# MCG-NKU/E2FGVI

Hardware: AMD Instinct MI355X
Metric: inpainted frames/sec at 432x240 T=10 (higher is better)
Workload: dtype f32; 1 GPU; BASELINE.json configs[1]: e2fgvi 432x240 T=10 l_t=10, 1 clip(s) per GPU per forward (1 in the job), random-init weights, torch.rand frames + box mask (SURVEY.md 8d); clips_per_gpu=1, precision=fp32, kernel_selection=e2fgvi_amd/tile_table.py (checked in, deterministic: ops.py), hip_graph=True, forwards_in_flight=2

## Files before the change

e2fgvi_amd/build.py:

```python
import os
import subprocess
import sys
from concurrent.futures import ThreadPoolExecutor

HERE = os.path.dirname(os.path.abspath(__file__))
CSRC = os.path.join(HERE, "csrc")
LIB = os.path.join(CSRC, "libe2fgvi_hip.so")
FLAGS = ["--offload-arch=gfx950", "-O3", "-std=c++17", "-fPIC", "-ffp-contract=fast"]
NOPK = ["-Xclang", "-target-feature", "-Xclang", "-packed-fp32-ops"]
UNITS = [("error.hip", "error.o", []), ("conv.hip", "conv.o", []), ("conv.hip", "conv_nopk.o", NOPK + ["-DE2_NOPK_VARIANT"]),
         ("conv_bf16x.hip", "conv_bf16x.o", NOPK), ("conv_wino.hip", "conv_wino.o", NOPK), ("conv_wino.hip", "conv_wino_x3.o", NOPK + ["-DE2_WINO_X3=1"]), ("conv_wino4.hip", "conv_wino4.o", NOPK), ("conv_tail.hip", "conv_tail.o", NOPK),
         ("mdcn.hip", "mdcn.o", NOPK), ("attention.hip", "attention.o", []),
         ("attention_bf16.hip", "attention_bf16.o", NOPK), ("attention_x3.hip", "attention_x3.o", NOPK), ("misc.hip", "misc.o", NOPK),
         ("video.hip", "video.o", NOPK), ("metrics.hip", "metrics.o", NOPK)]
NOPK_OBJECTS = ("conv_nopk.o", "conv_bf16x.o", "conv_wino.o", "conv_wino4.o", "conv_wino_x3.o", "conv_tail.o", "mdcn.o", "attention_bf16.o", "attention_x3.o", "misc.o", "video.o", "metrics.o")
OBJDUMP = "/opt/rocm/lib/llvm/bin/llvm-objdump"


def _hipcc():
    for c in (os.environ.get("HIPCC"), "/opt/rocm/bin/hipcc"):
        if c and os.path.exists(c):
            return c
    return "hipcc"


def _stale(out, deps):
    return (not os.path.exists(out)) or any(os.path.getmtime(d) > os.path.getmtime(out) for d in deps)


def build(force=False, verbose=False, nopk_all=False, lib=None, tag=None, defines=()):
    hipcc = _hipcc()
    if tag:
        nopk_all = False
    objdir = os.path.join(CSRC, ("build_" + tag) if tag else ("build_nopk" if nopk_all else "build"))
    os.makedirs(objdir, exist_ok=True)
    out = lib or (os.path.join(CSRC, "libe2fgvi_hip_%s.so" % tag) if tag else
                  os.path.join(CSRC, "libe2fgvi_hip_nopk.so") if nopk_all else LIB)
    headers = [os.path.join(CSRC, "common.h"), os.path.join(HERE, "..", "include", "e2fgvi_hip.h"), os.path.abspath(__file__)]
    jobs = []
    for src, obj, extra in UNITS:
        sp, op = os.path.join(CSRC, src), os.path.join(objdir, obj)
        if nopk_all and not any(f == "-packed-fp32-ops" for f in extra):
            extra = extra + NOPK
        if force or _stale(op, [sp] + headers):
            jobs.append([hipcc] + FLAGS + extra + list(defines) + ["-c", sp, "-o", op])

    def run(cmd):
        if verbose:
            print(" ".join(cmd), flush=True)
        subprocess.check_call(cmd)

    with ThreadPoolExecutor(max_workers=min(4, max(1, len(jobs)))) as ex:
        list(ex.map(run, jobs))
    objs = [os.path.join(objdir, obj) for _, obj, _ in UNITS]
    if force or jobs or _stale(out, objs):
        run([hipcc, "--offload-arch=gfx950", "-shared", "-fPIC", "-o", out] + objs)
    if jobs:
        verify_isa(objdir)
        if not nopk_all:
            verify_wino_waits(objdir)
            verify_exit_reuse(objdir)
            verify_no_scratch(objdir)
    return out


def build_variant(tag, *defines):
    return build(tag=tag, defines=defines)


def device_isa(obj):
    import shutil
    import tempfile
    d = tempfile.mkdtemp(prefix="e2isa")
    try:
        local = os.path.join(d, os.path.basename(obj))
        shutil.copy(obj, local)
        subprocess.run([OBJDUMP, "--offloading", os.path.basename(obj)], cwd=d, check=True, stdout=subprocess.DEVNULL,
                       stderr=subprocess.DEVNULL)
        dev = [f for f in os.listdir(d) if "gfx950" in f]
        if not dev:
            return ""
        return subprocess.run([OBJDUMP, "-d", os.path.join(d, dev[0])], check=True, capture_output=True, text=True).stdout
    finally:
        shutil.rmtree(d, ignore_errors=True)


def verify_isa(objdir=None):
    import re
    objdir = objdir or os.path.join(CSRC, "build")
    if not os.path.exists(OBJDUMP):
        return
    for obj in NOPK_OBJECTS:
        isa = device_isa(os.path.join(objdir, obj))
# ... 84 lines not shown
                                       % (obj, name[:60], ins[a][0], ins[b][0]))
            g = counts[0] - counts[1] if len(counts) > 1 else counts[0]
            if counts[-1] != 0 or g <= 0 or any(c != counts[0] - j * g for j, c in enumerate(counts)):
                raise RuntimeError("%s: %s: group waits %s are not (P-1) G, ..., G, 0" % (obj, name[:60], counts))
            tail = [k for k in list(range(inner[-1] + 2, hi + 1)) + list(range(lo, inner[0])) if vmem.match(ins[k][1])]
            planes = tail[-(counts[0] + g):]
            if len(planes) != counts[0] + g or any(ins[k][1] != "buffer_load_dwordx4" or " lds" in ins[k][2] for k in planes):
                raise RuntimeError("%s: %s: the %d vector-memory instructions in front of the group waits are not the plane "
                                   "loads" % (obj, name[:60], counts[0] + g))
            continue
        for j, m in enumerate(inner):
            n = int(re.search(r"vmcnt\((\d+)\)", ins[m][2]).group(1))
            if j:
                rng = range(inner[j - 1] + 2, m)
            else:
                rng = list(range(inner[-1] + 2, hi + 1)) + list(range(lo, m))
            cnt = sum(1 for k in rng if vmem.match(ins[k][1]))
            if cnt != n:
                raise RuntimeError("%s: %s: explicit s_waitcnt vmcnt(%d) at 0x%x follows %d vector-memory instructions "
                                   "since the previous explicit wait" % (obj, name[:60], n, ins[m][0], cnt))
    return loops


def verify_wino_waits(objdir=None, objects=("conv_wino.o", "conv_wino_x3.o", "conv_wino4.o")):
    objdir = objdir or os.path.join(CSRC, "build")
    if not os.path.exists(OBJDUMP):
        return 0
    loops = 0
    for obj in objects:
        for name, ins in _kernels(device_isa(os.path.join(objdir, obj))).items():
            loops += check_kernel_waits(obj, name, ins)
    if not loops:
        raise RuntimeError("verify_wino_waits: no K loop with marked waits found (disassembly format changed?)")
    return loops


def _vregs(text):
    import re
    r = set()
    for m in re.finditer(r"\bv\[(\d+):(\d+)\]", text):
        r.update(range(int(m.group(1)), int(m.group(2)) + 1))
    for m in re.finditer(r"\bv(\d+)\b", text):
        r.add(int(m.group(1)))
    return r


def _successors(ins, at):
    succ = []
    for i, (a, m, o) in enumerate(ins):
        if m in ("s_endpgm", "s_endpgm_saved"):
            succ.append(())
        elif m == "s_branch" or m.startswith("s_cbranch"):
            off = int(o.split()[0])
            off -= 65536 if off > 32767 else 0
            tgt = at.get(a + 4 + 4 * off)
            if tgt is None:
                raise RuntimeError("branch at 0x%x leaves the kernel" % a)
            succ.append((tgt,) if m == "s_branch" else (tgt, i + 1))
        elif m.startswith("s_setpc") or m.startswith("s_swappc"):
            raise RuntimeError("indirect jump at 0x%x: control flow cannot be followed" % a)
        else:
            succ.append((i + 1,) if i + 1 < len(ins) else ())
    return succ


def check_exit_reuse(obj, name, ins, min_mfma=8):
# ... 125 lines not shown
```

e2fgvi_amd/csrc/conv_bf16x.hip:

```cpp
#include "common.h"

namespace {

typedef __bf16 bf16x8 __attribute__((ext_vector_type(8)));
typedef unsigned int u32x4 __attribute__((ext_vector_type(4)));
typedef __attribute__((address_space(3))) void lds_void;

struct ConvXParams {
    const void* src[E2FGVI_MAX_SRC];
    int ld[E2FGVI_MAX_SRC];
    int coff[E2FGVI_MAX_SRC];
    int cpg[E2FGVI_MAX_SRC];
    unsigned src_bytes[E2FGVI_MAX_SRC];
    int nsrc;
    int N, H, W, Ho, Wo, KH, KW, stride, pad;
    int padx;
    int osy, osx, opy, opx, oH, oW;
    int res_bcast;
    int Cout, Cout_g, Npad;
    int M;
    int tilesM, tilesN;
    int nsteps;
    unsigned wgroup_bytes;
    long long wgroup_elems;
    const void* w;
    const float* bias;
    const void* res;
    int res_ld, res_coff, res_bf16;
    void* dst;
    int dst_ld, dst_coff, dst_bf16, dst_nchw;
    __bf16* dst2;
    int dst2_ld, dst2_coff;
    int split_from;
// ... 643 lines not shown
                for (int c = 0; c < 8; ++c) if (full || n + c < p.Cout_g) o[(long long)c * HoWo] = v[c];
            } else if (p.dst_bf16) {
                E16* o = reinterpret_cast<E16*>(p.dst) + dof;
                if (vec_d) *reinterpret_cast<e16x8*>(o) = hv;
                else {
#pragma unroll
                    for (int c = 0; c < 8; ++c) if (full || n + c < p.Cout_g) o[c] = hv[c];
                }
            } else {
                float* o = reinterpret_cast<float*>(p.dst) + dof;
                if (vec_d) {
                    f32x4 w0 = {v[0], v[1], v[2], v[3]}, w1 = {v[4], v[5], v[6], v[7]};
                    *reinterpret_cast<f32x4*>(o) = w0;
                    *reinterpret_cast<f32x4*>(o + 4) = w1;
                } else {
#pragma unroll
                    for (int c = 0; c < 8; ++c) if (full || n + c < p.Cout_g) o[c] = v[c];
                }
            }
            if (p.dst2 && !p.split_plane) {
                E16* o = reinterpret_cast<E16*>(p.dst2) + (long long)m * p.dst2_ld + p.dst2_coff + co;
                if (vec_2) *reinterpret_cast<e16x8*>(o) = hv;
                else {
#pragma unroll
                    for (int c = 0; c < 8; ++c) if (full || n + c < p.Cout_g) o[c] = hv[c];
                }
            }
        }
    }
    }
#endif
}

struct PackX {
    int Cout, groups, KH, KW, nsrc;
    int cpg[E2FGVI_MAX_SRC];
    int Cout_g, Npad, Cin_g, steps_per_tap;
    int kc, ch;
    int tp_cq;
    long long total, wgroup_elems;
};

bool geometry_x(int Cout, int groups, int KH, int KW, int nsrc, const int32_t* cpg, PackX* q, bool f32 = false) {
    q->kc = f32 ? 32 : 64;
    q->ch = f32 ? 4 : 8;
    q->tp_cq = 0;
    if (Cout <= 0 || groups <= 0 || Cout % groups || KH <= 0 || KW <= 0 || nsrc < 1 || nsrc > E2FGVI_MAX_SRC) return false;
    q->Cout = Cout; q->groups = groups; q->KH = KH; q->KW = KW; q->nsrc = nsrc;
    q->Cout_g = Cout / groups;
    q->Npad = round_up(q->Cout_g, 32);
    q->Cin_g = 0;
    q->steps_per_tap = 0;
    for (int s = 0; s < E2FGVI_MAX_SRC; ++s) q->cpg[s] = 0;
    for (int s = 0; s < nsrc; ++s) {
        if (cpg[s] <= 0 || cpg[s] % q->ch) return false;
        q->cpg[s] = cpg[s];
        q->Cin_g += cpg[s];
        q->steps_per_tap += cdiv(cpg[s], q->kc);
    }
    q->wgroup_elems = (long long)KH * KW * q->steps_per_tap * q->kc * q->Npad;
    q->total = q->wgroup_elems * groups;
    return true;
}

__device__ __forceinline__ float pack_value(const float* __restrict__ w, const PackX& p, int g, int step, int koct, int n, int e) {
    if (p.tp_cq) {
// ... 58 lines not shown
    p.tilesM = cdiv(p.M, BM);
    p.tilesN = cdiv(p.Cout_g, BN);
    if constexpr (PP) {
        if (mode != 2 || p.tp_cq) {
            e2fgvi_set_error("conv2d_x: the ping-pong tiles (107, 108) are for the split-operand mode without tap-packed weights");
            return E2FGVI_EUNSUP;
        }
        hipLaunchKernelGGL((conv_bf16x_kernel<BM, BN, WGM, WGN, false, 2, true>), dim3(p.tilesM * p.tilesN, groups, 1), dim3(64 * WGM * WGN), 0, st, p);
        E2_LAUNCH_CHECK("conv2d_x");
        return 0;
    } else {
    if (S3 && !(p.KH == 3 && p.KW == 3 && p.stride == 1 && p.pad == 1)) {
        e2fgvi_set_error("conv2d_x: the row-shift tiles (11..17) are for 3x3 stride-1 pad-1 layers");
        return E2FGVI_EINVAL;
    }
    if (mode == 1 || mode == 2) {
        if constexpr (!S3) {
            if (mode == 2)
                hipLaunchKernelGGL((conv_bf16x_kernel<BM, BN, WGM, WGN, false, 2>), dim3(p.tilesM * p.tilesN, groups, 1), dim3(64 * WGM * WGN), 0, st, p);
            else
                hipLaunchKernelGGL((conv_bf16x_kernel<BM, BN, WGM, WGN, false, 1>), dim3(p.tilesM * p.tilesN, groups, 1), dim3(64 * WGM * WGN), 0, st, p);
        } else {
            e2fgvi_set_error("conv2d_x: the row-shift tiles (11..18) take bf16 operands only");
            return E2FGVI_EUNSUP;
        }
    } else if (mode == 3) {
        hipLaunchKernelGGL((conv_bf16x_kernel<BM, BN, WGM, WGN, S3, 3>), dim3(p.tilesM * p.tilesN, groups, 1), dim3(64 * WGM * WGN), 0, st, p);
    } else {
        hipLaunchKernelGGL((conv_bf16x_kernel<BM, BN, WGM, WGN, S3, 0>), dim3(p.tilesM * p.tilesN, groups, 1), dim3(64 * WGM * WGN), 0, st, p);
    }
    E2_LAUNCH_CHECK("conv2d_x");
    return 0;
    }
}

}

static bool geometry_taps(int Cout, int KH, int KW, int cin, PackX* q, bool f32 = false) {
    const int32_t cpg[1] = {cin};
    if (cin > 56 || KW < 2 || !geometry_x(Cout, 1, KH, KW, 1, cpg, q, f32)) return false;
    q->tp_cq = cin / q->ch;
    const int steps = cdiv(KH * KW * q->tp_cq, 8);
    q->wgroup_elems = (long long)steps * q->kc * q->Npad;
    q->total = q->wgroup_elems;
    return true;
}

static int mode_x(const char* who, int32_t code) {
    switch (code) {
        case E2FGVI_BF16: return 0;
        case E2FGVI_F32: return 1;
        case E2FGVI_BF16X3: return 2;
        case E2FGVI_F16: return 3;
        default: break;
    }
    e2fgvi_set_error("%s: mode %d is none of E2FGVI_F32 (0), E2FGVI_BF16 (1), E2FGVI_BF16X3 (2), E2FGVI_F16 (3)", who, code);
    return -1;
}

static bool pack_geometry(const char* who, int mode, int tap_packed, int Cout, int groups, int KH, int KW, int nsrc,
                          const int32_t* src_cpg, PackX* q) {
    const bool f32 = mode == 1 || mode == 2;
    const int ch = f32 ? 4 : 8;
    if (!src_cpg) {
        e2fgvi_set_error("%s: null src_cpg", who);
        return false;
// ... 114 lines not shown
    if (d->tap_packed) {
        PackX qt;
        E2_REQUIRE(d->nsrc == 1 && d->groups == 1 && geometry_taps(d->Cout, d->KH, d->KW, d->src_cpg[0], &qt, f32), E2FGVI_EINVAL,
                   "conv2d_x: tap-packed weights are for one source of <= 56 channels, no groups, KW >= 2");
        E2_REQUIRE(d->tile < 10 || d->tile > 20, E2FGVI_EUNSUP, "conv2d_x: the row-shift tiles do not take tap-packed weights");
        q.wgroup_elems = qt.wgroup_elems;
        p.tp_cq = qt.tp_cq;
        p.tp_magic = 0xFFFFFFFFu / (unsigned)d->KW + 1u;
        p.tp_magic_cq = qt.tp_cq > 1 ? 0xFFFFFFFFu / (unsigned)qt.tp_cq + 1u : 0u;
        p.nsteps = cdiv(d->KH * d->KW * qt.tp_cq, 8);
    }
    p.wgroup_elems = q.wgroup_elems; p.wgroup_bytes = (unsigned)(q.wgroup_elems * wbytes_num);
    p.w = d->wpacked; p.bias = d->bias;
    p.res = d->residual; p.res_ld = d->res_ld; p.res_coff = d->res_coff; p.res_bf16 = d->res_dtype == dt16;
    p.dst = d->dst; p.dst_ld = d->dst_ld; p.dst_coff = d->dst_coff; p.dst_bf16 = d->dst_dtype == dt16;
    p.dst_nchw = d->dst_nchw;
    p.dst2 = (__bf16*)d->dst2; p.dst2_ld = d->dst2_ld; p.dst2_coff = d->dst2_coff;
    p.split_from = d->dst2_split_from; p.split_plane = d->dst2_plane_stride;
    p.act = d->act; p.slope = d->slope;
    hipStream_t st = (hipStream_t)stream;
    int tile = d->tile;
    p.dbg_noload = 0;
    if (tile == 21 || tile == 24 || tile == 26 || tile == 27) { p.dbg_noload = 1; tile -= 20; }
    if (tile == 31 || tile == 34 || tile == 36) { p.dbg_noload = 2; tile -= 30; }
    if (tile == 41 || tile == 44 || tile == 46) { p.dbg_noload = 3; tile -= 40; }
    if (tile == 61 || tile == 66) { p.dbg_noload = 8; tile -= 60; }
    if (tile == 71 || tile == 74 || tile == 76 || tile == 77) { p.dbg_noload = 16; tile -= 70; }
    if (tile == 81 || tile == 84 || tile == 86 || tile == 87) { p.dbg_noload = 32; tile -= 80; }
    if (!tile) {
        if (p.Cout_g <= 32) tile = 3;
        else if (p.Cout_g <= 64) tile = 2;
        else tile = ((long long)cdiv(p.M, 128) * cdiv(p.Cout_g, 128) * d->groups >= 384) ? 1 : 4;
    }
    switch (tile) {
        case 1: return launch_x<128, 128, 2, 2, false>(p, d->groups, st, mode);
        case 2: return launch_x<128, 64, 2, 2, false>(p, d->groups, st, mode);
        case 3: return launch_x<128, 32, 4, 1, false>(p, d->groups, st, mode);
        case 4: return launch_x<64, 128, 2, 2, false>(p, d->groups, st, mode);
        case 5: return launch_x<64, 64, 2, 2, false>(p, d->groups, st, mode);
        case 6: return launch_x<256, 128, 4, 2, false>(p, d->groups, st, mode);
        case 7: return launch_x<256, 256, 4, 2, false>(p, d->groups, st, mode);
        case 8: return launch_x<256, 192, 4, 2, false>(p, d->groups, st, mode);
        case 107: return launch_x<256, 256, 4, 2, false, true>(p, d->groups, st, mode);
        case 108: return launch_x<256, 192, 4, 2, false, true>(p, d->groups, st, mode);
        case 11: return launch_x<128, 128, 2, 2, true>(p, d->groups, st, mode);
        case 12: return launch_x<128, 64, 2, 2, true>(p, d->groups, st, mode);
        case 13: return launch_x<128, 32, 4, 1, true>(p, d->groups, st, mode);
        case 14: return launch_x<64, 128, 2, 2, true>(p, d->groups, st, mode);
        case 16: return launch_x<256, 128, 4, 2, true>(p, d->groups, st, mode);
        case 17: return launch_x<256, 256, 4, 2, true>(p, d->groups, st, mode);
        case 18: return launch_x<256, 64, 4, 2, true>(p, d->groups, st, mode);
        default: break;
    }
    e2fgvi_set_error("conv2d_x: unknown tile %d", tile);
    return E2FGVI_EINVAL;
}

extern "C" int e2fgvi_conv2d_x(const e2fgvi_convx_desc* d, int32_t mode, void* stream) {
    const int m = mode_x("conv2d_x", mode);
    return m < 0 ? E2FGVI_EINVAL : conv2d_x(d, stream, m);
}
```

e2fgvi_amd/lib.py:

```python
import ctypes as C
import os

_HERE = os.path.dirname(os.path.abspath(__file__))
LIB_PATH = os.environ.get("E2FGVI_LIB") or os.path.join(_HERE, "csrc", "libe2fgvi_hip.so")

ABI_VERSION = 9
MAX_SRC = 4
ACT_NONE, ACT_RELU, ACT_LRELU, ACT_TANH, ACT_DCNPOST = 0, 1, 2, 3, 4
DT_F32, DT_BF16 = 0, 1
DT_BF16X3 = 2
DT_F16 = 3

_fp = C.c_void_p


class ConvDesc(C.Structure):
    _fields_ = [
        ("src", _fp * MAX_SRC), ("src_ld", C.c_int32 * MAX_SRC), ("src_coff", C.c_int32 * MAX_SRC),
        ("src_cpg", C.c_int32 * MAX_SRC), ("nsrc", C.c_int32),
        ("N", C.c_int32), ("H", C.c_int32), ("W", C.c_int32), ("Ho", C.c_int32), ("Wo", C.c_int32),
        ("KH", C.c_int32), ("KW", C.c_int32), ("stride", C.c_int32), ("pad", C.c_int32),
        ("groups", C.c_int32), ("Cout", C.c_int32), ("bk", C.c_int32),
        ("wpacked", _fp), ("bias", _fp), ("residual", _fp), ("res_ld", C.c_int32), ("res_coff", C.c_int32),
        ("dst", _fp), ("dst_ld", C.c_int32), ("dst_coff", C.c_int32), ("dst_nchw", C.c_int32),
# ... 12 lines not shown
        ("res_dtype", C.c_int32),
        ("dst", _fp), ("dst_ld", C.c_int32), ("dst_coff", C.c_int32), ("dst_dtype", C.c_int32),
        ("dst2", _fp), ("dst2_ld", C.c_int32), ("dst2_coff", C.c_int32),
        ("act", C.c_int32), ("slope", C.c_float), ("tile", C.c_int32), ("dst_nchw", C.c_int32), ("tap_packed", C.c_int32),
        ("out_grid", C.c_int32), ("pad_left", C.c_int32),
        ("out_sy", C.c_int32), ("out_sx", C.c_int32), ("out_py", C.c_int32), ("out_px", C.c_int32),
        ("out_H", C.c_int32), ("out_W", C.c_int32), ("res_bcast", C.c_int32),
        ("dst2_split_from", C.c_int32), ("dst2_plane_stride", C.c_int64),
    ]


class MdcnDesc(C.Structure):
    _fields_ = [
        ("src", _fp * 2), ("src_ld", C.c_int32 * 2), ("src_c", C.c_int32 * 2), ("nsrc", C.c_int32),
        ("N", C.c_int32), ("H", C.c_int32), ("W", C.c_int32), ("Ho", C.c_int32), ("Wo", C.c_int32),
        ("KH", C.c_int32), ("KW", C.c_int32), ("stride", C.c_int32), ("pad", C.c_int32), ("dil", C.c_int32),
        ("deform_groups", C.c_int32), ("Cout", C.c_int32),
        ("offset", _fp), ("off_ld", C.c_int32), ("mask", _fp), ("mask_ld", C.c_int32),
        ("flows", _fp), ("max_residue", C.c_float),
        ("wpacked", _fp), ("bias", _fp),
        ("dst", _fp), ("dst_ld", C.c_int32), ("dst_coff", C.c_int32), ("tile", C.c_int32), ("dst_dtype", C.c_int32),
        ("mfma_dtype", C.c_int32), ("src_dtype", C.c_int32), ("src_planar", C.c_int32),
    ]


_i32, _i64, _f = C.c_int32, C.c_int64, C.c_float
SYMBOLS = {
    "e2fgvi_last_error": (C.c_char_p, []),
    "e2fgvi_abi_version": (C.c_int, []),
    "e2fgvi_nhwc_to_planar16": (C.c_int, [_fp, _fp, _i64, _i32, _fp]),
    "e2fgvi_conv2d_nhwc": (C.c_int, [C.POINTER(ConvDesc), _fp]),
    "e2fgvi_conv2d_nhwc_nopk": (C.c_int, [C.POINTER(ConvDesc), _fp]),
    "e2fgvi_conv2d_x": (C.c_int, [C.POINTER(ConvXDesc), _i32, _fp]),
    "e2fgvi_packed_conv_weight_x_size": (_i64, [_i32, _i32, _i32, _i32, _i32, _i32, _i32, C.POINTER(_i32)]),
    "e2fgvi_pack_conv_weight_x": (C.c_int, [_fp, _fp, _i32, _i32, _i32, _i32, _i32, _i32, _i32, C.POINTER(_i32), _fp]),
    "e2fgvi_packed_conv_weight_size": (_i64, [_i32, _i32, _i32, _i32, _i32, C.POINTER(_i32), _i32]),
    "e2fgvi_pack_conv_weight": (C.c_int, [_fp, _fp, _i32, _i32, _i32, _i32, _i32, C.POINTER(_i32), _i32, _fp]),
    "e2fgvi_packed_winograd_weight_size": (_i64, [_i32, _i32, _i32, C.POINTER(_i32)]),
    "e2fgvi_pack_winograd_weight": (C.c_int, [_fp, _fp, _i32, _i32, _i32, C.POINTER(_i32), _fp]),
    "e2fgvi_conv3x3_winograd": (C.c_int, [C.POINTER(ConvDesc), _fp]),
    "e2fgvi_packed_winograd_weight_x3_size": (_i64, [_i32, _i32, _i32, C.POINTER(_i32)]),
    "e2fgvi_pack_winograd_weight_x3": (C.c_int, [_fp, _fp, _i32, _i32, _i32, C.POINTER(_i32), _fp]),
    "e2fgvi_conv3x3_winograd_x3": (C.c_int, [C.POINTER(ConvDesc), _fp]),
    "e2fgvi_packed_winograd4_weight_size": (_i64, [_i32, _i32, _i32, C.POINTER(_i32), _i32]),
    "e2fgvi_pack_winograd4_weight": (C.c_int, [_fp, _fp, _i32, _i32, _i32, C.POINTER(_i32), _i32, _fp]),
    "e2fgvi_conv3x3_winograd4": (C.c_int, [C.POINTER(ConvDesc), _i32, _fp]),
    "e2fgvi_packed_tail_weight_size": (_i64, [_i32, _i32]),
    "e2fgvi_pack_tail_weight": (C.c_int, [_fp, _fp, _i32, _i32, _i32, _fp]),
    "e2fgvi_conv3x3_tail": (C.c_int, [_fp, _i32, _i32, _fp, _fp, _fp, _i32, _i32, _i32, _i32, C.c_float, _fp]),
    "e2fgvi_mdcn_nhwc": (C.c_int, [C.POINTER(MdcnDesc), _fp]),
    "e2fgvi_packed_dcn_weight_size": (_i64, [_i32, _i32, _i32, _i32, _i32]),
    "e2fgvi_pack_dcn_weight": (C.c_int, [_fp, _fp, _i32, _i32, _i32, _i32, _i32, _i32, _fp]),
    "e2fgvi_focal_attention": (C.c_int, [_fp, _fp, _fp, _i32, _fp, _fp, _i32, _i32, _i32, _i32, _i32, _fp]),
    "e2fgvi_split3_kv": (C.c_int, [_fp, _fp, _i64, _fp]),
    "e2fgvi_focal_attention_x3": (C.c_int, [_fp, _fp, _fp, _i32, _fp, _fp, _i32, _i32, _i32, _i32, _i32, _fp]),
    "e2fgvi_nchw_to_nhwc": (C.c_int, [_fp, _fp, _i32, _i32, _i32, _i32, _i32, _i32, _f, _f, _fp]),
    "e2fgvi_nhwc_to_nchw": (C.c_int, [_fp, _i32, _fp, _i32, _i32, _i32, _i32, _fp]),
    "e2fgvi_resize_bilinear": (C.c_int, [_fp, _i32, _i32, _i32, _fp, _i32, _i32, _i32, _i32, _i32, _i32, _i32, _i32, _fp, _fp, _fp]),
    "e2fgvi_avgpool2_nhwc": (C.c_int, [_fp, _fp, _i32, _i32, _i32, _i32, _fp]),
    "e2fgvi_spynet_level_input": (C.c_int, [_fp, _fp, _fp, _fp, _fp, _fp, _i32, _i32, _i32, _i32, _fp]),
    "e2fgvi_prop_cond": (C.c_int, [_fp, _i32, _fp, _i32, _i32, _fp, _fp, _i64, _fp, _i32, _fp, _fp, _i32, _i32, _i32, _i32, _fp]),
    "e2fgvi_layernorm": (C.c_int, [_fp, _fp, _fp, _fp, _i32, _i64, _i32, _fp]),
    "e2fgvi_window_pool": (C.c_int, [_fp, _i32, _fp, _fp, _fp, _i32, _i32, _i32, _i32, _fp]),
    "e2fgvi_ffn_fold": (C.c_int, [_fp, _fp, _i32, _i32, _i32, _i32, _i32, _i32, _i32, _i32, _fp]),
    "e2fgvi_ffn_unfold": (C.c_int, [_fp, _fp, _i32, _i32, _i32, _i32, _i32, _i32, _i32, _i32, _fp]),
    "e2fgvi_mask_prepare": (C.c_int, [_fp, _i32, _i32, _i32, _fp, _fp, _fp, _i32, _i32, _i32, _fp]),
# ... 120 lines not shown
```

e2fgvi_amd/ops.py:

```python
import collections
import ctypes as C
import math
import os

import torch

from . import lib as _L

ACT_NONE, ACT_RELU, ACT_LRELU, ACT_TANH, ACT_DCNPOST = _L.ACT_NONE, _L.ACT_RELU, _L.ACT_LRELU, _L.ACT_TANH, _L.ACT_DCNPOST


def _stream():
    return C.c_void_p(torch.cuda.current_stream().cuda_stream)


def _chk(t, name, dtype=torch.float32):
    if not isinstance(t, torch.Tensor) or not t.is_cuda:
        raise TypeError("%s must be a CUDA (ROCm) tensor -- the HIP path has no CPU fallback" % name)
    if t.dtype != dtype:
        raise TypeError("%s must be %s, got %s" % (name, dtype, t.dtype))
    if not t.is_contiguous():
        raise ValueError("%s must be contiguous" % name)
    return t


def _ptr(t):
    return C.c_void_p(t.data_ptr()) if t is not None else C.c_void_p(0)


def empty_nhwc(n, h, w, c, device):
    return torch.empty((n, h, w, c), dtype=torch.float32, device=device)


TUNE_CANDIDATES = (0, 213, 223, 211, 219, 216)
WINO_CANDIDATES = (64, 132, 164, 32)
W4_CODES = {2464: (2, 64)}
_W4_MINPIX = 20000
XTUNE_CANDIDATES = (1, 4, 6, 7, 8, 2, 5, 3, 107, 108)
XTUNE_ROWSHIFT = (11, 16, 17, 12, 13, 18)
X3_ENABLED = os.environ.get("E2FGVI_X3", "1") != "0"
X3_MARGIN = 0.97
X3_BASE = 30000
W3_BASE = 40000
W3_CANDIDATES = (132, 164, 32, 5132, 6064)
W3_WIDE = 6064
W3_WIDE_FALLBACK = 164
DMA_BASE = 2000


def _decode(code):
    if code >= W3_BASE:
        return "w3", code - W3_BASE
    if code >= X3_BASE:
        return "x3", code - X3_BASE
    if code in W4_CODES:
        return "w4", code
    if DMA_BASE <= code < DMA_BASE + 100:
        return "dma", code - DMA_BASE
    return "own", code


_TUNED = {}
AUTOTUNE = os.environ.get("E2FGVI_AUTOTUNE", "0") == "1"
TUNE_REPS = max(1, int(os.environ.get("E2FGVI_TUNE_REPS", "1") or 1))
TABLE_FORMAT = 2
_SIZE_FIELD = 8


def _default_tune_file():
    try:
        st = os.stat(_L.LIB_PATH)
        d = os.environ.get("E2FGVI_CACHE_DIR") or os.path.join(os.path.dirname(os.path.abspath(__file__)), ".tile_cache")
        os.makedirs(d, exist_ok=True)
        dev = "gpu"
        if torch.cuda.is_available():
# ... 514 lines not shown


def _dt_key(t):
    return _L.DT_BF16 if t.dtype == torch.float16 else _dt(t)


def _chk_any(t, name):
    if not isinstance(t, torch.Tensor) or not t.is_cuda:
        raise TypeError("%s must be a CUDA (ROCm) tensor -- the HIP path has no CPU fallback" % name)
    if not t.is_contiguous():
        raise ValueError("%s must be contiguous" % name)
    _dt(t)
    return t


class PackedConvX(_ConvLayer):

    _NCHW_ERROR = "NCHW out must be fp32 %(want)s"

    def __init__(self, weight, bias, cpg, groups=1, stride=1, pad=0, dtype=torch.bfloat16, taps=None, x3=False):
        lib = _L.load()
        w = self._init_layer(weight, bias, cpg, groups, stride, pad)
        self.dtype = dtype
        self.f32 = dtype == torch.float32
        self.x3 = bool(x3)
        if self.x3 and not self.f32:
            raise ValueError("x3 splitting is for fp32 sources")
        self.f16 = dtype == torch.float16
        if not self.f32 and dtype not in HALF16:
            raise TypeError("PackedConvX: dtype must be float32, bfloat16 or float16")
        self._mode = mode = _L.DT_BF16X3 if self.x3 else _DT_CODE[dtype]
        conv2d_x = lib.e2fgvi_conv2d_x
        self._fn = lambda desc_ref, stream: conv2d_x(desc_ref, mode, stream)
        self._w_raw = w if (self.f32 and not self.x3) else None
        self._taps_arg = taps
        self.taps = (len(self.cpg) == 1 and groups == 1 and self.cpg[0] <= 56 and self.KW > 1
                     and (taps is True if self.f32 else taps is not False))
        self._wdtype = torch.bfloat16 if self.x3 else dtype
        self._wp = None
        if self._w_raw is None:
            self._wp = self._pack(w)
        else:
            _L.check(min(0, int(lib.e2fgvi_packed_conv_weight_x_size(*self._wgeom()))), "packed_conv_weight_x_size")

    @property
    def wpacked(self):
        return _lazy(vars(self), "_wp", self.name + " (LDS-DMA GEMM weights)", lambda: self._pack(self._w_raw))

    def weight_bytes(self):
        return (0 if self._wp is None else self._wp.numel() * self._wp.element_size()) + (self.alt3.weight_bytes() if self.alt3 is not None else 0)

    def _wgeom(self):
        return self._mode, int(self.taps), self.Cout, self.groups, self.KH, self.KW, len(self.cpg), self._cpg_arr()

    def _pack(self, w):
        lib = _L.load()
        return _pack_weights(lib.e2fgvi_packed_conv_weight_x_size, lib.e2fgvi_pack_conv_weight_x, w, self._wdtype, "conv_weight_x",
                             *self._wgeom())

    def _alt3(self):
        if self._w_raw is None:
            return self.alt3
        return _lazy(vars(self), "alt3", self.name + " (split-operand GEMM alternative)",
                     lambda: self._x_alternative(taps=self._taps_arg, x3=True))

    def _desc(self, srcs, out, out_coff, residual, res_coff, act, slope, out2, out_nchw):
# ... 844 lines not shown
```

include/e2fgvi_hip.h:

```cpp
#ifndef E2FGVI_HIP_H
#define E2FGVI_HIP_H

#include <stdint.h>

#ifdef __cplusplus
extern "C" {
#endif

#define E2FGVI_EINVAL (-1)
#define E2FGVI_EUNSUP (-2)

#define E2FGVI_ACT_NONE 0
#define E2FGVI_ACT_RELU 1
#define E2FGVI_ACT_LRELU 2
#define E2FGVI_ACT_TANH 3
int e2fgvi_mask_prepare(const uint8_t* masks, int32_t L, int32_t Hin, int32_t Win, const int32_t* ytab, const int32_t* xtab,
                        uint8_t* out, int32_t H, int32_t W, int32_t iterations, void* stream);
int e2fgvi_masked_clip(const uint8_t* frames, const uint8_t* masks, const int32_t* ids, int32_t t, int32_t H, int32_t W,
                       float* clip, int32_t Hp, int32_t Wp, void* stream);
int e2fgvi_composite(const float* pred, const int32_t* ids, const uint8_t* first, int32_t n, const uint8_t* frames,
                     const uint8_t* masks, float* comp, int32_t H, int32_t W, int32_t Hp, int32_t Wp, void* stream);
int e2fgvi_resample_u8(const uint8_t* src, uint8_t* dst, int32_t L, int32_t H, int32_t W, int32_t n_out, int32_t axis,
                       const int32_t* bounds, const int32_t* coeffs, int32_t ksize, void* stream);
int e2fgvi_resample_rows_u8(const uint8_t* src, uint8_t* dst, int32_t L, int32_t H, int32_t W, int32_t n_out, int32_t row0,
// ... 150 lines not shown
int e2fgvi_cast(const void* src, int32_t src_dtype, void* dst, int32_t dst_dtype, int64_t n, void* stream);

typedef struct {
    const void* src[E2FGVI_MAX_SRC];
    int32_t src_ld[E2FGVI_MAX_SRC];
    int32_t src_coff[E2FGVI_MAX_SRC];
    int32_t src_cpg[E2FGVI_MAX_SRC];
    int32_t nsrc;
    int32_t N, H, W, Ho, Wo;
    int32_t KH, KW, stride, pad;
    int32_t groups;
    int32_t Cout;
    const void* wpacked;
    const float* bias;
    const void* residual;
    int32_t res_ld, res_coff, res_dtype;
    void* dst;
    int32_t dst_ld, dst_coff, dst_dtype;
    void* dst2;
    int32_t dst2_ld, dst2_coff;
    int32_t act;
    float slope;
    int32_t tile;
    int32_t dst_nchw;
    int32_t tap_packed;
    int32_t out_grid, pad_left;
    int32_t out_sy, out_sx, out_py, out_px, out_H, out_W;
    int32_t res_bcast;
    int32_t dst2_split_from;
    int64_t dst2_plane_stride;
} e2fgvi_convx_desc;

int e2fgvi_conv2d_x(const e2fgvi_convx_desc* d, int32_t mode, void* stream);
int64_t e2fgvi_packed_conv_weight_x_size(int32_t mode, int32_t tap_packed, int32_t Cout, int32_t groups, int32_t KH, int32_t KW,
                                         int32_t nsrc, const int32_t* src_cpg);
int e2fgvi_pack_conv_weight_x(const float* w, void* wpacked, int32_t mode, int32_t tap_packed, int32_t Cout, int32_t groups,
                              int32_t KH, int32_t KW, int32_t nsrc, const int32_t* src_cpg, void* stream);

int e2fgvi_conv3x3_winograd_x3(const e2fgvi_conv_desc* d, void* stream);
int64_t e2fgvi_packed_winograd_weight_x3_size(int32_t Cout, int32_t groups, int32_t nsrc, const int32_t* src_cpg);
int e2fgvi_pack_winograd_weight_x3(const float* w, void* wpacked, int32_t Cout, int32_t groups, int32_t nsrc,
                                   const int32_t* src_cpg, void* stream);

int e2fgvi_split3_kv(const float* qkv_rows, void* planes, int64_t rows, void* stream);
int e2fgvi_focal_attention_x3(const float* qkv, const void* planes, const int32_t* key_tab, int32_t tab_ld, const int32_t* nkeys,
                              float* out, int32_t B, int32_t T, int32_t fh, int32_t fw, int32_t waves, void* stream);

int e2fgvi_focal_attention_16(const void* qkv, const void* kv_pool, const int32_t* key_tab, int32_t tab_ld,
                              const int32_t* nkeys, void* out, int32_t dtype, int32_t B, int32_t T, int32_t fh, int32_t fw,
                              void* stream);
int e2fgvi_focal_attention_16_variant(int variant);

#ifdef __cplusplus
}
#endif
#endif
```

Before: 925.4 frames/s.

## Add halo-tiled 7x7 conv kernel staging input patch once in LDS

Adds a dedicated kernel for 7x7 stride-1 pad-3 convolutions on 32 or 64 input channels in the bf16x3 split mode. Each block loads its output tile plus a 3-pixel halo once, splits it into three bf16 planes in LDS, and reuses that patch for all 49 taps. Weights stream through a 2- or 3-stage DMA pipeline with counted waits. This is meant to avoid re-gathering im2col input per tap from global memory, at the cost of a specialised code path with its own layout, dispatch conditions and ISA wait verification.

Result: no change. 931.9 frames/s (median of 6 runs) (+0.7%).

```diff
diff --git a/e2fgvi_amd/build.py b/e2fgvi_amd/build.py
--- a/e2fgvi_amd/build.py
+++ b/e2fgvi_amd/build.py
@@ -36,7 +36,8 @@
     os.makedirs(objdir, exist_ok=True)
     out = lib or (os.path.join(CSRC, "libe2fgvi_hip_%s.so" % tag) if tag else
                   os.path.join(CSRC, "libe2fgvi_hip_nopk.so") if nopk_all else LIB)
-    headers = [os.path.join(CSRC, "common.h"), os.path.join(HERE, "..", "include", "e2fgvi_hip.h"), os.path.abspath(__file__)]
+    headers = [os.path.join(CSRC, "common.h"), os.path.join(CSRC, "conv7_halo_map.h"), os.path.join(HERE, "..", "include", "e2fgvi_hip.h"),
+               os.path.abspath(__file__)]
     jobs = []
     for src, obj, extra in UNITS:
         sp, op = os.path.join(CSRC, src), os.path.join(objdir, obj)
@@ -59,6 +60,7 @@
         verify_isa(objdir)
         if not nopk_all:
             verify_wino_waits(objdir)
+            verify_halo7_waits(objdir)
             verify_exit_reuse(objdir)
             verify_no_scratch(objdir)
     return out
@@ -209,6 +211,28 @@
             loops += check_kernel_waits(obj, name, ins)
     if not loops:
         raise RuntimeError("verify_wino_waits: no K loop with marked waits found (disassembly format changed?)")
+    return loops
+
+
+def verify_halo7_waits(objdir=None, obj="conv_bf16x.o"):
+    objdir = objdir or os.path.join(CSRC, "build")
+    if not os.path.exists(OBJDUMP):
+        return 0
+    loops, kernels = 0, 0
+    for name, ins in _kernels(device_isa(os.path.join(objdir, obj))).items():
+        if "conv7_halo_kernel" not in name:
+            continue
+        kernels += 1
+        if any(m.startswith("scratch_") for _, m, _ in ins):
+            raise RuntimeError("%s: %s uses scratch memory" % (obj, name[:60]))
+        k = check_kernel_waits(obj, name, ins)
+        counted = any(m == "s_waitcnt" and "vmcnt" in o and "vmcnt(0)" not in o and i + 1 < len(ins) and ins[i + 1][1:] == (m, o)
+                      for i, (_, m, o) in enumerate(ins))
+        if counted and not k:
+            raise RuntimeError("%s: %s: marked waits but no K loop around them (disassembly format changed?)" % (obj, name[:60]))
+        loops += k
+    if kernels != 4 or not loops:
+        raise RuntimeError("verify_halo7_waits: %d conv7_halo_kernel instantiations, %d checked loops in %s" % (kernels, loops, obj))
     return loops
 
 
diff --git a/e2fgvi_amd/csrc/conv7_halo_map.h b/e2fgvi_amd/csrc/conv7_halo_map.h
--- /dev/null
+++ b/e2fgvi_amd/csrc/conv7_halo_map.h
@@ -0,0 +1,46 @@
+#pragma once
+
+#if defined(__HIPCC__)
+#define E2_HALO7_HD __host__ __device__ __forceinline__
+#else
+#define E2_HALO7_HD inline
+#endif
+
+template <int CODE, int CIN>
+struct Halo7Map {
+    static_assert((CODE == 3 || CODE == 5) && (CIN == 32 || CIN == 64), "tile codes 3 / 5 on 32 / 64 input channels");
+    static constexpr int NT = 256;
+    static constexpr int BH = 8, BW = CODE == 3 ? 16 : 8;
+    static constexpr int BN = CODE == 3 ? 32 : 64;
+    static constexpr int WGN = BN / 32, WGM = 4 / WGN;
+    static constexpr int PH = BH + 6, PW = BW + 6;
+    static constexpr int CQ = CIN / 8;
+    static constexpr int P = CQ + 1;
+    static constexpr int RP = (PW * P + (CODE == 3 ? 15 : 7)) / 16 * 16 + (CODE == 3 ? 0 : 8);
+    static constexpr int PLANE_SLOTS = PH * RP, PLANE_BYTES = PLANE_SLOTS * 16;
+    static constexpr int A_BYTES = 3 * PLANE_BYTES;
+    static constexpr int UNITS = PH * PW * CQ;
+    static constexpr int U_IT = (UNITS + NT - 1) / NT;
+    static constexpr int KSTEPS_PER_TAP = CIN / 32;
+    static constexpr int B_STEP = BN * 12 * 16;
+    static constexpr int NS = (A_BYTES + 2 * B_STEP) * 2 <= 160 * 1024 ? 2 : 3;
+    static constexpr int SMEM = A_BYTES + NS * B_STEP;
+    static constexpr int PPW = CODE == 3 ? 2 : 3;
+    static_assert(RP >= PW * P && RP % 16 == (CODE == 3 ? 0 : 8) && SMEM <= 160 * 1024, "plane layout");
+
+    static E2_HALO7_HD bool unit(int u, int& py, int& px, int& cq) {
+        const int pix = u / CQ;
+        cq = u - pix * CQ;
+        py = pix / PW;
+        px = pix - py * PW;
+        return u < UNITS;
+    }
+    static E2_HALO7_HD int slot(int py, int px, int cq) { return py * RP + px * P + cq; }
+    static E2_HALO7_HD int b_item(int wave, int j) { return (CODE == 3 ? (j == 0 ? wave : 4 + (wave >> 1)) : wave + 4 * j) * 64; }
+    static E2_HALO7_HD void pixel(int wm, int i, int& ty, int& tx) {
+        const int t = wm * 32 + i;
+        ty = t / BW;
+        tx = t - ty * BW;
+    }
+    static E2_HALO7_HD int frag_slot(int ty, int tx, int ky, int kx, int blk, int q) { return slot(ty + ky, tx + kx, blk * 4 + q); }
+};
diff --git a/e2fgvi_amd/csrc/conv_bf16x.hip b/e2fgvi_amd/csrc/conv_bf16x.hip
--- a/e2fgvi_amd/csrc/conv_bf16x.hip
+++ b/e2fgvi_amd/csrc/conv_bf16x.hip
@@ -1,4 +1,7 @@
+#include <type_traits>
+
 #include "common.h"
+#include "conv7_halo_map.h"
 
 namespace {
 
@@ -708,6 +711,228 @@
 #endif
 }
 
+template <int N> __device__ __forceinline__ void halo7_wait_barrier() {
+    __builtin_amdgcn_sched_barrier(0);
+    if constexpr (N > 0)
+        asm volatile("s_waitcnt vmcnt(%0)\n\ts_waitcnt vmcnt(%0)\n\ts_waitcnt lgkmcnt(0)\n\ts_barrier" :: "n"(N) : "memory");
+    else
+        asm volatile("s_waitcnt vmcnt(0) lgkmcnt(0)\n\ts_barrier" ::: "memory");
+    __builtin_amdgcn_sched_barrier(0);
+}
+
+template <int CODE, int CIN>
+__global__ __launch_bounds__(256) void conv7_halo_kernel(const ConvXParams p) {
+#if defined(__HIP_DEVICE_COMPILE__)
+    typedef Halo7Map<CODE, CIN> MAP;
+    constexpr int BW = MAP::BW, BN = MAP::BN, WGN = MAP::WGN, NS = MAP::NS, B_STEP = MAP::B_STEP;
+    constexpr int A_BYTES = MAP::A_BYTES, PLANE = MAP::PLANE_BYTES;
+    constexpr int PPW = MAP::PPW;
+    constexpr int LDE = 36, EPI = 4 * 32 * LDE * 4;
+    constexpr unsigned OOB = 0xFFFFFFFFu;
+    static_assert(EPI <= MAP::SMEM, "epilogue region");
+
+    __shared__ __attribute__((aligned(1024))) unsigned char smem[MAP::SMEM];
+
+    const int tid = threadIdx.x;
+    const int lane = tid & 63, wave = __builtin_amdgcn_readfirstlane(tid >> 6);
+    const int wm = wave / WGN, wn = wave % WGN;
+    const int i = lane & 31, h = lane >> 5;
+    const int tilesX = (p.Wo + BW - 1) / BW, tilesY = (p.Ho + 7) / 8;
+    const int logical = xcd_remap(blockIdx.x, p.tilesM * p.tilesN);
+    const int tile_m = logical / p.tilesN, tile_n = logical - tile_m * p.tilesN;
+    const int img = tile_m / (tilesY * tilesX);
+    const int trem = tile_m - img * (tilesY * tilesX);
+    const int y0 = (trem / tilesX) * 8, x0 = (trem % tilesX) * BW;
+    const int n0 = tile_n * BN;
+
+    const unsigned smem_lds = (unsigned)(unsigned long long)(lds_void*)smem;
+    const pp_i32x4 wrsrc = pp_rsrc_words(p.w, p.wgroup_bytes);
+    const unsigned b_step = 12u * (unsigned)p.Npad * 16u;
+    int b_item[PPW];
+    unsigned b_off[PPW];
+#pragma unroll
+    for (int j = 0; j < PPW; ++j) {
+        b_item[j] = MAP::b_item(wave, j);
+        const int item = b_item[j] + lane;
+        const int koct = item / BN, n = item - koct * BN;
+        b_off[j] = (n0 + n) < p.Npad ? (unsigned)((koct * p.Npad + n0 + n) * 16) : OOB;
+    }
+    auto issue_piece = [&](int slot, int step, int j) __attribute__((always_inline)) {
+        const unsigned dst = (unsigned)__builtin_amdgcn_readfirstlane((int)(smem_lds + (unsigned)(A_BYTES + slot * B_STEP + b_item[j] * 16)));
+        pp_dma16(wrsrc, dst, b_off[j], (unsigned)__builtin_amdgcn_readfirstlane((int)((unsigned)step * b_step)));
+    };
+    auto issue_b = [&](int slot, int step) __attribute__((always_inline)) {
+#pragma unroll
+        for (int j = 0; j < PPW; ++j) issue_piece(slot, step, j);
+    };
+#pragma unroll
+    for (int s = 0; s < NS; ++s) issue_b(s, s);
+
+    {
+        const __amdgpu_buffer_rsrc_t arsrc = make_rsrc(p.src[0], p.src_bytes[0]);
+        const unsigned ld4 = (unsigned)p.ld[0] * 4u, ch4 = (unsigned)p.coff[0] * 4u;
+        f32x4 v[MAP::U_IT][2];
+#pragma unroll
+        for (int it = 0; it < MAP::U_IT; ++it) {
+            int py, px, cq;
+            const bool in = MAP::unit(tid + it * MAP::NT, py, px, cq);
+            const int iy = y0 - 3 + py, ix = x0 - 3 + px;
+            const bool ok = in && (unsigned)iy < (unsigned)p.H && (unsigned)ix < (unsigned)p.W;
+            const unsigned off = (unsigned)((img * p.H + iy) * p.W + ix) * ld4 + ch4 + (unsigned)cq * 32u;
+            v[it][0] = __builtin_bit_cast(f32x4, __builtin_amdgcn_raw_buffer_load_b128(arsrc, (int)(ok ? off : OOB), 0, 0));
+            v[it][1] = __builtin_bit_cast(f32x4, __builtin_amdgcn_raw_buffer_load_b128(arsrc, (int)(ok ? off + 16u : OOB), 0, 0));
+        }
+#pragma unroll
+        for (int it = 0; it < MAP::U_IT; ++it) {
+            int py, px, cq;
+            if (!MAP::unit(tid + it * MAP::NT, py, px, cq)) continue;
+            bf16x8 hi, mid, lo;
+            split8(v[it][0], v[it][1], hi, mid, lo);
+            unsigned char* o = smem + MAP::slot(py, px, cq) * 16;
+            *reinterpret_cast<bf16x8*>(o) = hi;
+            *reinterpret_cast<bf16x8*>(o + PLANE) = mid;
+            *reinterpret_cast<bf16x8*>(o + 2 * PLANE) = lo;
+        }
+    }
+    asm volatile("s_waitcnt vmcnt(0)" ::: "memory");
+    __syncthreads();
+
+    f32x16 acc;
+#pragma unroll
+    for (int r = 0; r < 16; ++r) acc[r] = 0.f;
+
+    int ty, tx;
+    MAP::pixel(wm, i, ty, tx);
+    const int a_lane = (MAP::slot(ty, tx, 0) + h) * 16;
+    const int b_lane = (h * BN + wn * 32 + i) * 16;
+    auto a_step = [&](int step) -> int {
+        const int tap = CIN == 64 ? step >> 1 : step, blk = CIN == 64 ? step & 1 : 0;
+        const int ky = (tap * 37) >> 8, kx = tap - ky * 7;
+        return MAP::frag_slot(0, 0, ky, kx, blk, 0) * 16;
+    };
+    bf16x8 fa[2][3], fb[2][3];
+    auto read = [&](int kk, int step, int slot) __attribute__((always_inline)) {
+        const unsigned char* a = smem + a_lane + a_step(step) + kk * 32;
+        const unsigned char* b = smem + A_BYTES + slot * B_STEP + b_lane + kk * (2 * BN * 16);
+#pragma unroll
+        for (int pl = 0; pl < 3; ++pl) {
+            fa[kk][pl] = *reinterpret_cast<const bf16x8*>(a + pl * PLANE);
+            fb[kk][pl] = *reinterpret_cast<const bf16x8*>(b + pl * (4 * BN * 16));
+        }
+        __builtin_amdgcn_sched_barrier(0);
+    };
+    auto mma = [&](int kk, int t0, int t1) __attribute__((always_inline)) {
+        constexpr int AI[6] = {2, 0, 1, 1, 0, 0}, BI[6] = {0, 2, 1, 0, 1, 0};
+#pragma unroll
+        for (int t = t0; t < t1; ++t) acc = __builtin_amdgcn_mfma_f32_32x32x16_bf16(fa[kk][AI[t]], fb[kk][BI[t]], acc, 0, 0, 0);
+        __builtin_amdgcn_sched_barrier(0);
+    };
+    auto kstep = [&](int step, int slot, int nslot, auto issue_tag, auto wait_tag, auto last_tag) __attribute__((always_inline)) {
+        constexpr bool ISSUE = decltype(issue_tag)::value, LAST = decltype(last_tag)::value;
+        constexpr int WAIT = decltype(wait_tag)::value;
+        mma(0, 0, 1);
+        read(1, step, slot);
+        mma(0, 1, 6);
+        mma(1, 0, 1);
+        if constexpr (!LAST) {
+            halo7_wait_barrier<WAIT>();
+            read(0, step + 1, nslot);
+        }
+        if constexpr (ISSUE) {
+#pragma unroll
+            for (int j = 0; j < PPW; ++j) {
+                mma(1, 1 + j, 2 + j);
+                issue_piece(slot, step + NS, j);
+                __builtin_amdgcn_sched_barrier(0);
+            }
+            mma(1, 1 + PPW, 6);
+        } else {
+            mma(1, 1, 6);
+        }
+    };
+    typedef std::integral_constant<bool, true> yes_t;
+    typedef std::integral_constant<bool, false> no_t;
+    const int nsteps = p.nsteps;
+    int slot = 0, step = 0;
+    read(0, 0, 0);
+#pragma unroll 1
+    for (; step < nsteps - NS; ++step) {
+        const int nslot = slot + 1 == NS ? 0 : slot + 1;
+        kstep(step, slot, nslot, yes_t(), std::integral_constant<int, (NS - 2) * PPW>(), no_t());
+        slot = nslot;
+    }
+    if constexpr (NS == 3) {
+        const int nslot = slot + 1 == NS ? 0 : slot + 1;
+        kstep(step, slot, nslot, no_t(), std::integral_constant<int, PPW>(), no_t());
+        slot = nslot;
+        ++step;
+    }
+    {
+        const int nslot = slot + 1 == NS ? 0 : slot + 1;
+        kstep(step, slot, nslot, no_t(), std::integral_constant<int, 0>(), no_t());
+        slot = nslot;
+        ++step;
+    }
+    kstep(step, slot, slot, no_t(), std::integral_constant<int, 0>(), yes_t());
+    __syncthreads();
+
+    float* E = reinterpret_cast<float*>(smem) + wave * (32 * LDE);
+#pragma unroll
+    for (int r = 0; r < 16; ++r) E[((r & 3) + 8 * (r >> 2) + 4 * h) * LDE + i] = acc[r];
+    __syncthreads();
+    const int col0 = (lane & 3) * 8;
+    const int n = n0 + wn * 32 + col0;
+    if (n >= p.Cout_g) return;
+    const bool full = n + 7 < p.Cout_g;
+    float bv[8];
+#pragma unroll
+    for (int c = 0; c < 8; ++c) bv[c] = (p.bias && (full || n + c < p.Cout_g)) ? p.bias[n + c] : 0.f;
+    const bool vec_d = full && ((p.dst_ld | p.dst_coff | n) & 7) == 0;
+    const bool vec_r = full && p.res && ((p.res_ld | p.res_coff | n) & 7) == 0;
+    const bool fast_n = (n0 + wn * 32 + 32 <= p.Cout_g) && p.act <= E2FGVI_ACT_LRELU && ((p.dst_ld | p.dst_coff) & 7) == 0 &&
+                        (!p.res || ((p.res_ld | p.res_coff) & 7) == 0);
+    const float neg = p.act == E2FGVI_ACT_RELU ? 0.f : (p.act == E2FGVI_ACT_LRELU ? p.slope : 1.f);
+#pragma unroll 1
+    for (int ps = 0; ps < 2; ++ps) {
+        const int row = ps * 16 + (lane >> 2);
+        int py, px;
+        MAP::pixel(wm, row, py, px);
+        const int oy = y0 + py, ox = x0 + px;
+        if (oy >= p.Ho || ox >= p.Wo) continue;
+        const int m = (img * p.Ho + oy) * p.Wo + ox;
+        const long long mr = p.res_bcast ? (long long)(oy * p.Wo + ox) : (long long)m;
+        const bool fast = fast_n && (m & ~31) + 32 <= p.M;
+        const f32x4 v0 = *reinterpret_cast<const f32x4*>(E + row * LDE + col0);
+        const f32x4 v1 = *reinterpret_cast<const f32x4*>(E + row * LDE + col0 + 4);
+        float v[8] = {v0[0], v0[1], v0[2], v0[3], v1[0], v1[1], v1[2], v1[3]};
+#pragma unroll
+        for (int c = 0; c < 8; ++c) v[c] += bv[c];
+        if (p.res) {
+            const float* rp = reinterpret_cast<const float*>(p.res) + mr * p.res_ld + p.res_coff + n;
+            if (vec_r) {
+                const f32x4 q0 = *reinterpret_cast<const f32x4*>(rp), q1 = *reinterpret_cast<const f32x4*>(rp + 4);
+#pragma unroll
+                for (int c = 0; c < 4; ++c) { v[c] += q0[c]; v[4 + c] += q1[c]; }
+            } else {
+#pragma unroll
+                for (int c = 0; c < 8; ++c) if (full || n + c < p.Cout_g) v[c] += rp[c];
+            }
+        }
+#pragma unroll
+        for (int c = 0; c < 8; ++c) v[c] = fast ? (v[c] > 0.f ? v[c] : v[c] * neg) : apply_act(v[c], p.act, p.slope);
+        float* o = reinterpret_cast<float*>(p.dst) + (long long)m * p.dst_ld + p.dst_coff + n;
+        if (vec_d) {
+            const f32x4 w0 = {v[0], v[1], v[2], v[3]}, w1 = {v[4], v[5], v[6], v[7]};
+            *reinterpret_cast<f32x4*>(o) = w0;
+            *reinterpret_cast<f32x4*>(o + 4) = w1;
+        } else {
+#pragma unroll
+            for (int c = 0; c < 8; ++c) if (full || n + c < p.Cout_g) o[c] = v[c];
+        }
+    }
+#endif
+}
+
 struct PackX {
     int Cout, groups, KH, KW, nsrc;
     int cpg[E2FGVI_MAX_SRC];
@@ -832,6 +1057,20 @@
     E2_LAUNCH_CHECK("conv2d_x");
     return 0;
     }
+}
+
+int g_conv7_halo = 1;
+long long g_conv7_halo_launches = 0;
+
+template <int CODE, int CIN>
+int launch_halo7(ConvXParams& p, hipStream_t st) {
+    typedef Halo7Map<CODE, CIN> MAP;
+    p.tilesM = p.N * cdiv(p.Ho, MAP::BH) * cdiv(p.Wo, MAP::BW);
+    p.tilesN = cdiv(p.Cout_g, MAP::BN);
+    hipLaunchKernelGGL((conv7_halo_kernel<CODE, CIN>), dim3(p.tilesM * p.tilesN, 1, 1), dim3(MAP::NT), 0, st, p);
+    E2_LAUNCH_CHECK("conv2d_x");
+    ++g_conv7_halo_launches;
+    return 0;
 }
 
 }
@@ -1012,6 +1251,13 @@
         else if (p.Cout_g <= 64) tile = 2;
         else tile = ((long long)cdiv(p.M, 128) * cdiv(p.Cout_g, 128) * d->groups >= 384) ? 1 : 4;
     }
+    if (g_conv7_halo && mode == 2 && !p.dbg_noload && (tile == 3 || tile == 5) && d->KH == 7 && d->KW == 7 && d->stride == 1 &&
+        d->pad == 3 && d->groups == 1 && d->nsrc == 1 && !d->tap_packed && !d->out_grid && !d->dst_nchw && !d->dst2 &&
+        (d->src_cpg[0] == 32 || d->src_cpg[0] == 64) && d->dst_dtype == E2FGVI_F32 && (!d->residual || d->res_dtype == E2FGVI_F32) &&
+        d->act != E2FGVI_ACT_DCNPOST) {
+        if (tile == 3) return d->src_cpg[0] == 32 ? launch_halo7<3, 32>(p, st) : launch_halo7<3, 64>(p, st);
+        return d->src_cpg[0] == 32 ? launch_halo7<5, 32>(p, st) : launch_halo7<5, 64>(p, st);
+    }
     switch (tile) {
         case 1: return launch_x<128, 128, 2, 2, false>(p, d->groups, st, mode);
         case 2: return launch_x<128, 64, 2, 2, false>(p, d->groups, st, mode);
@@ -1040,3 +1286,11 @@
     const int m = mode_x("conv2d_x", mode);
     return m < 0 ? E2FGVI_EINVAL : conv2d_x(d, stream, m);
 }
+
+extern "C" int64_t e2fgvi_conv7_halo_launches(void) { return g_conv7_halo_launches; }
+
+extern "C" int e2fgvi_set_conv7_halo(int on) {
+    const int prev = g_conv7_halo;
+    g_conv7_halo = on ? 1 : 0;
+    return prev;
+}
diff --git a/e2fgvi_amd/lib.py b/e2fgvi_amd/lib.py
--- a/e2fgvi_amd/lib.py
+++ b/e2fgvi_amd/lib.py
@@ -68,6 +68,8 @@
     "e2fgvi_conv2d_nhwc": (C.c_int, [C.POINTER(ConvDesc), _fp]),
     "e2fgvi_conv2d_nhwc_nopk": (C.c_int, [C.POINTER(ConvDesc), _fp]),
     "e2fgvi_conv2d_x": (C.c_int, [C.POINTER(ConvXDesc), _i32, _fp]),
+    "e2fgvi_set_conv7_halo": (C.c_int, [C.c_int]),
+    "e2fgvi_conv7_halo_launches": (_i64, []),
     "e2fgvi_packed_conv_weight_x_size": (_i64, [_i32, _i32, _i32, _i32, _i32, _i32, _i32, C.POINTER(_i32)]),
     "e2fgvi_pack_conv_weight_x": (C.c_int, [_fp, _fp, _i32, _i32, _i32, _i32, _i32, _i32, _i32, C.POINTER(_i32), _fp]),
     "e2fgvi_packed_conv_weight_size": (_i64, [_i32, _i32, _i32, _i32, _i32, C.POINTER(_i32), _i32]),
diff --git a/e2fgvi_amd/ops.py b/e2fgvi_amd/ops.py
--- a/e2fgvi_amd/ops.py
+++ b/e2fgvi_amd/ops.py
@@ -41,6 +41,15 @@
 X3_ENABLED = os.environ.get("E2FGVI_X3", "1") != "0"
 X3_MARGIN = 0.97
 X3_BASE = 30000
+HALO7 = os.environ.get("E2FGVI_HALO7", "1") != "0"
+
+
+def set_halo7(on):
+    global HALO7
+    HALO7 = bool(on)
+    return bool(_L.load().e2fgvi_set_conv7_halo(int(HALO7)))
+
+
 W3_BASE = 40000
 W3_CANDIDATES = (132, 164, 32, 5132, 6064)
 W3_WIDE = 6064
@@ -621,6 +630,8 @@
         self._mode = mode = _L.DT_BF16X3 if self.x3 else _DT_CODE[dtype]
         conv2d_x = lib.e2fgvi_conv2d_x
         self._fn = lambda desc_ref, stream: conv2d_x(desc_ref, mode, stream)
+        if not HALO7:
+            lib.e2fgvi_set_conv7_halo(0)
         self._w_raw = w if (self.f32 and not self.x3) else None
         self._taps_arg = taps
         self.taps = (len(self.cpg) == 1 and groups == 1 and self.cpg[0] <= 56 and self.KW > 1
diff --git a/include/e2fgvi_hip.h b/include/e2fgvi_hip.h
--- a/include/e2fgvi_hip.h
+++ b/include/e2fgvi_hip.h
@@ -206,6 +206,8 @@
 } e2fgvi_convx_desc;
 
 int e2fgvi_conv2d_x(const e2fgvi_convx_desc* d, int32_t mode, void* stream);
+int e2fgvi_set_conv7_halo(int on);
+int64_t e2fgvi_conv7_halo_launches(void);
 int64_t e2fgvi_packed_conv_weight_x_size(int32_t mode, int32_t tap_packed, int32_t Cout, int32_t groups, int32_t KH, int32_t KW,
                                          int32_t nsrc, const int32_t* src_cpg);
 int e2fgvi_pack_conv_weight_x(const float* w, void* wpacked, int32_t mode, int32_t tap_packed, int32_t Cout, int32_t groups,
```
